# zhan-xu/MoRig

Hardware: AMD Instinct MI355X
Metric: meshes/sec jointnet_motion forward, 4 k-vert synthetic (higher is better)
Workload: dtype f32 (split-fp16: 3x f16 MFMA, f32 accumulate); 1 GPU; jointnet_motion(num_keyframes=5, attn) eval forward, B=64 x 4096-vertex synthetic meshes/GPU, BASELINE.json configs[1]; step=COO->CSR prep + forward, meshes_per_gpu=64, global_batch=64, vertices_per_mesh=4096, parallelism=mesh-sharded dp1, guard_read=deferred, geo_graph=device

## Files before the change

morig_amd/csrc/dma_ring.h:

```cpp
#pragma once
#include "mfma_types.h"

namespace morig {

template <int MT, int NT> struct SplitFrag { f16x8 ah[MT], al[MT], bh[NT], bl[NT]; };

template <int MT, int NT>
__device__ __forceinline__ void load_split_frag(SplitFrag<MT, NT>& f, const char* st, int aoff, int boff, int s2, int hi, int x7) {
    const int sh = ((2 * s2 + hi) ^ x7) * 16, sl = ((4 + 2 * s2 + hi) ^ x7) * 16;
#pragma unroll
    for (int mt = 0; mt < MT; ++mt) {
        f.ah[mt] = *reinterpret_cast<const f16x8*>(st + aoff + mt * 32 * 128 + sh);
        f.al[mt] = *reinterpret_cast<const f16x8*>(st + aoff + mt * 32 * 128 + sl);
    }
#pragma unroll
    for (int nt = 0; nt < NT; ++nt) {
        f.bh[nt] = *reinterpret_cast<const f16x8*>(st + boff + nt * 32 * 128 + sh);
        f.bl[nt] = *reinterpret_cast<const f16x8*>(st + boff + nt * 32 * 128 + sl);
    }
}

template <bool SWAP>
__device__ __forceinline__ void split_mm(const f16x8& x, const f16x8& w, f32x16& c) {
    if constexpr (SWAP) c = __builtin_amdgcn_mfma_f32_32x32x16_f16(w, x, c, 0, 0, 0);
// ... 32 lines not shown
}
__device__ __forceinline__ void dma_piece(const char* base, int c, unsigned o, char* st, int piece) {
    asm volatile("" : "+v"(o));
    __builtin_amdgcn_global_load_lds((glb_void_t*)(base + c * 128 + o), (lds_void_t*)(st + piece * 1024), 16, 0, 0);
}

__device__ __forceinline__ f32x16 acc_zero() {
    f32x16 v;
#pragma unroll
    for (int r = 0; r < 16; ++r) v[r] = 0.f;
    return v;
}
__device__ __forceinline__ f32x16 acc_from_panel(const float* pn, int nt) {
    f32x16 v;
#pragma unroll
    for (int g4 = 0; g4 < 4; ++g4) {
        const f32x4 b4 = *reinterpret_cast<const f32x4*>(pn + nt * 32 + 8 * g4);
#pragma unroll
        for (int q = 0; q < 4; ++q) v[4 * g4 + q] = b4[q];
    }
    return v;
}

}
```

morig_amd/csrc/epilogue_store.h:

```cpp
#pragma once
#include <hip/hip_runtime.h>
#include <type_traits>

namespace morig {

template <int NT, int SLAB = 32, int PAD = 4> struct EpilogueTile {
    static constexpr int CW = NT * 32, LDT = CW + PAD, FLOATS = SLAB * LDT;
};

template <int MT, int NT, bool ALLOW16, class P, int SLAB = 32, int PAD = 4>
__device__ __forceinline__ void store_tile_transposed(const P& p, f32x16 (&acc)[MT][NT], float* T, const int* sseg,
                                                      int rl_base, int row0, int Mlim, int colw0, int lane) {
    static_assert(SLAB == 32 || SLAB == 16, "slab = whole or half MFMA row tile");
    constexpr int CW = EpilogueTile<NT, SLAB, PAD>::CW, LDT = EpilogueTile<NT, SLAB, PAD>::LDT;
    constexpr int VW = 4, LPR = CW / VW, RPI = 64 / LPR;
    constexpr int VW16 = 8, LPR16 = CW / VW16, RPI16 = 64 / LPR16;
    constexpr int NV = ALLOW16 ? 8 : 4;
    const int l31 = lane & 31, hi = lane >> 5;
    const bool y16 = ALLOW16 && p.y16 != 0;
    const bool vec_ok = (reinterpret_cast<size_t>(p.Y) & 15) == 0 && (p.ldy & 3) == 0;
    const int cg = y16 ? (lane % LPR16) * VW16 : (lane % LPR) * VW;
    const int rsel = y16 ? lane / LPR16 : lane / LPR;
    const int col0 = colw0 + cg;
    const int nv = y16 ? VW16 : VW;
// ... 195 lines not shown
        }
    }
    if (ovf) *p.ovf = 1;
}

template <int MT, int NT, class P>
__device__ __forceinline__ void store_tile_regs(const P& p, f32x16 (&acc)[MT][NT], const float* ps, const float* pt,
                                                int rl_base, int row0, int Mlim, int colw0, int cl0, int lane, bool rb_slow) {
#ifdef MORIG_EPI_GENERIC
    store_tile_regs_t<MT, NT, P, false, false, false, false>(p, acc, ps, pt, rl_base, row0, Mlim, colw0, cl0, lane, rb_slow);
#else
    if (rb_slow) { store_tile_regs_t<MT, NT, P, false, false, false, false>(p, acc, ps, pt, rl_base, row0, Mlim, colw0, cl0, lane, rb_slow); return; }
    const int key = (p.y16 != 0 ? 1 : 0) | (p.relu != 0 ? 2 : 0) | (ps != nullptr ? 4 : 0);
#define MORIG_EPI_CASE(K, Y, R, A) case K: store_tile_regs_t<MT, NT, P, true, Y, R, A>(p, acc, ps, pt, rl_base, row0, Mlim, colw0, cl0, lane, false); break;
    switch (key) {
        MORIG_EPI_CASE(0, false, false, false) MORIG_EPI_CASE(1, true, false, false) MORIG_EPI_CASE(2, false, true, false)
        MORIG_EPI_CASE(3, true, true, false) MORIG_EPI_CASE(4, false, false, true) MORIG_EPI_CASE(5, true, false, true)
        MORIG_EPI_CASE(6, false, true, true) MORIG_EPI_CASE(7, true, true, true)
    }
#undef MORIG_EPI_CASE
#endif
}

}
```

morig_amd/csrc/gemm_dma.hip:

```cpp
#include "common.h"
#include "dma_ring.h"
#include "epilogue_store.h"
#include "pool_epilogue.h"
#include <stdlib.h>

namespace morig {

template <int BM, int BN, int NT, int DMA_NS, bool TR = false, bool TAIL = false>
__global__ __launch_bounds__((BM / 64) * (BN / (32 * NT)) * 64) void gemm16_dma_kernel(const GemmDmaParams p) {
    constexpr int MT = 2;
    constexpr int WNW = BN / (32 * NT);
    constexpr int NW = (BM / 64) * WNW;
    constexpr int DMA_STAGE = (BM + BN) * 128;
    constexpr int XJ = BM / 8 / NW, WJ = BN / 8 / NW;
    constexpr int PER_CHUNK = XJ + WJ;
    constexpr int TBYTES = NW * EpilogueTile<NT>::FLOATS * 4;
    constexpr int RING = DMA_NS * DMA_STAGE;
    constexpr int SM0 = (TR || RING > TBYTES) ? RING : TBYTES;
    constexpr int PANEL = TR ? 3 * BN * 4 : 0;
    __shared__ __attribute__((aligned(128))) char smem[SM0 + BM * 4 + PANEL];
    int* sseg = reinterpret_cast<int*>(smem + SM0);
    float* pan = reinterpret_cast<float*>(smem + SM0 + BM * 4);

    const int tid = threadIdx.x, lane = tid & 63, wave = tid >> 6;
    const int l31 = lane & 31, hi = lane >> 5;
    const int wm = wave / WNW, wn = wave % WNW;
    const int lin = xcd_remap(blockIdx.x, gridDim.x);
    const int tn = lin % p.tiles_n, tm = lin / p.tiles_n;
    const int row0 = tm * BM;

#ifdef MORIG_DMA_TRACE
#define DMA_TS(k) do { if ((int)blockIdx.x == (int)(gridDim.x / 2 + 8) && lane == 0) p.trace[(k) * 8 + wave] = __builtin_readcyclecounter(); } while (0)
// ... 79 lines not shown
    const int aoff = (wm * 64 + l31) * 128, boff = BM * 128 + (wn * NT * 32 + l31) * 128;
#ifndef MORIG_2MFMA
    constexpr bool LOHI = true;
#else
    constexpr bool LOHI = false;
#endif
    typedef SplitFrag<MT, NT> Frag;
    auto load_frag = [&](Frag& f, int c, int s2) { load_split_frag(f, smem + (c % DMA_NS) * DMA_STAGE, aoff, boff, s2, hi, x7); };
    auto mma = [&](const Frag& f) { split_mma<TR, LOHI>(f, acc); };
    auto wait_chunk = [&](int c) {
        int younger = nchunk - 1 - c;
        if (younger > DMA_NS - 2) younger = DMA_NS - 2;
        static_assert(DMA_NS >= 2 && DMA_NS <= 4, "ring depth");
        if (younger == 2) asm volatile("s_waitcnt vmcnt(%0)" ::"n"(2 * PER_CHUNK) : "memory");
        else if (younger == 1) asm volatile("s_waitcnt vmcnt(%0)" ::"n"(PER_CHUNK) : "memory");
        else asm volatile("s_waitcnt vmcnt(0)" ::: "memory");
    };
    auto mma_pair = [&](const Frag& f, int mt, int nt0) __attribute__((always_inline)) { split_mma_pair<TR, LOHI>(f, acc, mt, nt0); };
    auto issue_one = [&](int c, int j) __attribute__((always_inline)) {
        char* st = smem + (c % DMA_NS) * DMA_STAGE;
        if (j < XJ) dma_x(st, c, j);
        else dma_w(st, c, j - XJ);
    };
    Frag f0, f1;
    wait_chunk(0);
    if constexpr (TR) asm volatile("s_waitcnt lgkmcnt(0)" ::: "memory");
    __builtin_amdgcn_s_barrier();
    if (DMA_NS - 1 < nchunk) issue(DMA_NS - 1);
    if constexpr (TR) {
#pragma unroll
        for (int nt = 0; nt < NT; ++nt) {
            const f32x16 v = acc_from_panel(pan + wn * NT * 32 + 4 * hi, nt);
#pragma unroll
            for (int mt = 0; mt < MT; ++mt) acc[mt][nt] = v;
        }
    }
    load_frag(f0, 0, 0);
#ifdef MORIG_DMA_BURST
    constexpr bool SPREAD = false;
#else
    constexpr bool SPREAD = (NT == 4 && MT == 2 && PER_CHUNK == 8);
#endif
    for (int c = 0; c < nchunk; ++c) {
        load_frag(f1, c, 1);
        mma(f0);
        const bool more = c + 1 < nchunk;
// ... 31 lines not shown
        if (rfirst >= p.M) return;
        pool_tile<MT, NT>(p, acc, rfirst, colw0, lane);
        return;
    }
    if constexpr (TR) {
        if (p.dbg & 1) { if (acc[0][0][0] == 12345.678f) p.Y[0] = 1.f; return; }
        DMA_TS(2);
        store_tile_regs<MT, NT>(p, acc, p.scale ? pan + BN : nullptr, pan + 2 * BN, wm * 64, row0, p.M, colw0, wn * NT * 32, lane, rb_slow);
        DMA_TS(3);
        return;
    }
    __syncthreads();
    if (p.dbg & 1) { if (acc[0][0][0] == 12345.678f) p.Y[0] = 1.f; return; }
    DMA_TS(2);
    store_tile_transposed<MT, NT, true>(p, acc, reinterpret_cast<float*>(smem) + wave * EpilogueTile<NT>::FLOATS, sseg,
                                        wm * 64, row0, p.M, colw0, lane);
    DMA_TS(3);
#ifdef MORIG_DMA_TRACE
    asm volatile("s_waitcnt vmcnt(0)" ::: "memory");
    DMA_TS(4);
#endif
}

int launch_gemm16_dma(const GemmDmaParams& p0, int tiles_m128, hipStream_t s) {
    GemmDmaParams p = p0;
    p.dbg = debug_flags();
    static const int mode = [] { const char* e = getenv("MORIG_DMA_TILE"); return e ? atoi(e) : 256; }();
    static const int persist = [] { const char* e = getenv("MORIG_DMA_PERSIST"); return e ? (e[0] == '0' ? 0 : 2) : 1; }();
    const bool deep_wide = p.pool != nullptr || (p.K >= 768 && p.N >= 1024);
    const bool vec_ok = p.pool != nullptr ||
                        ((reinterpret_cast<uintptr_t>(p.Y) & 15) == 0 && (p.ldy & 3) == 0 &&
                         (!p.rowbias || ((reinterpret_cast<uintptr_t>(p.rowbias) & 15) == 0 && (p.ld_rowbias & 3) == 0)));
    if (p.Xt && !(mode == 256 && p.N % 256 == 0 && !p.pool)) return MORIG_E_UNSUPPORTED;
    static const int small_tiles = [] { const char* e = getenv("MORIG_DMA_SMALL_TILES"); return e ? atoi(e) : 256; }();
    const bool few_tiles = !p.Xt && p.N % 256 == 0 && (long)cdiv(p.M, 256) * (p.N / 256) <= small_tiles;
    if (!few_tiles && !p.Xt && mode == 256 && p.N % 256 == 0 && p.K > 32 && vec_ok && (persist == 2 || (persist == 1 && deep_wide))) {
        if (!p.pool) prof_retag(K_GEMM16_DMAP);
        return launch_gemm16_dmap(p0, s);
    }
    if (mode == 256 && p.N % 256 == 0 && !few_tiles) {
        p.tiles_n = p.N / 256;
        const int nb = cdiv(p.M, 256) * p.tiles_n;
#ifdef MORIG_DMA_TRACE
        static unsigned long long* trace_buf = [] { void* b = nullptr; return hipMalloc(&b, 64 * 8) == hipSuccess ? (unsigned long long*)b : nullptr; }();
        p.trace = trace_buf;
#endif
        static const bool want_tr = [] { const char* e = getenv("MORIG_GEMM_TR"); return !(e && e[0] == '0'); }();
        const bool tr = want_tr && !p.pool && (reinterpret_cast<uintptr_t>(p.Y) & 15) == 0 && (p.ldy & 3) == 0 &&
                        (!p.rowbias || ((reinterpret_cast<uintptr_t>(p.rowbias) & 15) == 0 && (p.ld_rowbias & 3) == 0));
        static const int shortk = [] { const char* e = getenv("MORIG_DMA_SHORTK"); return e ? atoi(e) : 0; }();
        if (tr && !p.Xt && shortk > 0 && p.K <= shortk && p.N % 128 == 0) {
            p.tiles_n = p.N / 128;
            const int nb128 = cdiv(p.M, 128) * p.tiles_n;
            prof_retag(K_GEMM16_DMA128);
            hipLaunchKernelGGL((gemm16_dma_kernel<128, 128, 2, 2, true>), dim3(nb128), dim3(256), 0, s, p);
            MORIG_LAUNCH_CHECK();
            return MORIG_OK;
        }
        if (p.Xt && !tr) return MORIG_E_UNSUPPORTED;
        if (p.Xt)    hipLaunchKernelGGL((gemm16_dma_kernel<256, 256, 4, 2, true, true>), dim3(nb), dim3(512), 0, s, p);
        else if (tr) hipLaunchKernelGGL((gemm16_dma_kernel<256, 256, 4, 2, true>), dim3(nb), dim3(512), 0, s, p);
        else         hipLaunchKernelGGL((gemm16_dma_kernel<256, 256, 4, 2, false>), dim3(nb), dim3(512), 0, s, p);
#ifdef MORIG_DMA_TRACE
        {
            unsigned long long h[64];
            if (hipStreamSynchronize(s) == hipSuccess && hipMemcpy(h, p.trace, sizeof(h), hipMemcpyDeviceToHost) == hipSuccess) {
                fprintf(stderr, "DMA_TRACE K=%d N=%d:", p.K, p.N);
                for (int w = 0; w < 8; w += 3) { fprintf(stderr, " w%d", w); for (int q = 1; q < 5; ++q) fprintf(stderr, " %lld", (long long)(h[q * 8 + w] - h[(q - 1) * 8 + w])); }
                fprintf(stderr, "\n");
            }
        }
#endif
    } else {
        p.tiles_n = cdiv(p.N, 128);
        prof_retag(K_GEMM16_DMA128);
        hipLaunchKernelGGL((gemm16_dma_kernel<128, 128, 2, 2, false>), dim3(tiles_m128 * p.tiles_n), dim3(256), 0, s, p);
    }
    MORIG_LAUNCH_CHECK();
    return MORIG_OK;
}

}
```

morig_amd/csrc/gemm_dmap.hip:

```cpp
#include "common.h"
#include "dma_ring.h"
#include "epilogue_store.h"
#include "pool_epilogue.h"
#include "pool_runs.h"
#include <stdlib.h>
#include <type_traits>

namespace morig {

struct GemmDmaHot { int M, K, ldx, ldw, tiles_n; const float* X; const float* W; const int* seg; };
typedef __attribute__((address_space(4))) const GemmDmaParams* kernarg_params_t;
template <bool POOL>
__global__ __launch_bounds__(512) void gemm16_dmap_kernel(const GemmDmaParams) {
#if defined(__HIP_DEVICE_COMPILE__)
    kernarg_params_t q = (kernarg_params_t)__builtin_amdgcn_kernarg_segment_ptr();
    asm volatile("" : "+s"(q));
    const GemmDmaHot p = {q->M, q->K, q->ldx, q->ldw, q->tiles_n, q->X, q->W, q->seg};
    constexpr int BM = 256, BN = 256, NT = 4, MT = 2;
    constexpr int WNW = BN / (32 * NT);
    constexpr int NW = (BM / 64) * WNW;
    constexpr int STAGE = (BM + BN) * 128;
    constexpr int XJ = BM / 8 / NW, WJ = BN / 8 / NW;
    constexpr int PANEL = 3 * BN;
    constexpr int PAIR = 2 * NT * 64;
    __shared__ __attribute__((aligned(128))) char smem[2 * STAGE + (POOL ? NW * PAIR * 4 : 2 * PANEL * 4)];
    float* pan = reinterpret_cast<float*>(smem + 2 * STAGE);

    const int tid = threadIdx.x, lane = tid & 63, wave = tid >> 6;
    const int l31 = lane & 31, hi = lane >> 5;
    const int wm = wave / WNW, wn = wave % WNW;

    const int tiles_m = (p.M + BM - 1) / BM;
    const int T = tiles_m * p.tiles_n;
    const int xcd = blockIdx.x & 7, bi = blockIdx.x >> 3, nbx = gridDim.x >> 3;
    TileList tl = {};
    int run_u = 0, run_left = 0;
// ... 91 lines not shown
            asm volatile("" : "+v"(f0.ah[0]), "+v"(f0.al[0]), "+v"(f0.ah[1]), "+v"(f0.al[1]));
            asm volatile("" : "+v"(f0.bh[0]), "+v"(f0.bl[0]), "+v"(f0.bh[1]), "+v"(f0.bl[1]), "+v"(f0.bh[2]), "+v"(f0.bl[2]), "+v"(f0.bh[3]), "+v"(f0.bl[3]));
#else
            load_frag(f0, st ^ 1, 0);
#endif
        }
        unsigned o0 = ox[0], o1 = ox[1], o2 = ox[2], o3 = ox[3];
        if (go && reclamp) { o0 = x_offset(0, nrow0); o1 = x_offset(1, nrow0); o2 = x_offset(2, nrow0); o3 = x_offset(3, nrow0); }
        mma_pair(f1, 0, 0); __builtin_amdgcn_sched_barrier(0);
        if constexpr (go) { dma_x(xb, o0, cc, st, 0); dma_x(xb, o1, cc, st, 1); }
        __builtin_amdgcn_sched_barrier(0);
        mma_pair(f1, 0, 2); __builtin_amdgcn_sched_barrier(0);
        if constexpr (go) { dma_x(xb, o2, cc, st, 2); dma_x(xb, o3, cc, st, 3); }
        __builtin_amdgcn_sched_barrier(0);
        mma_pair(f1, 1, 0); __builtin_amdgcn_sched_barrier(0);
        if constexpr (go) { dma_w(wb, cc, st, 0); dma_w(wb, cc, st, 1); }
        __builtin_amdgcn_sched_barrier(0);
        mma_pair(f1, 1, 2); __builtin_amdgcn_sched_barrier(0);
        if constexpr (go) { dma_w(wb, cc, st, 2); dma_w(wb, cc, st, 3); }
        __builtin_amdgcn_sched_barrier(0);
    };
    typedef std::integral_constant<int, 1> Yes;
    typedef std::integral_constant<int, 0> No;

    int lin = tl.first;
    if constexpr (POOL) {
        lin = pool_run_first_tile(run_u, p.tiles_n, q->run);
        run_left = pool_run_count(run_u, tiles_m, p.tiles_n, q->run) - 1;
    }
    static_assert(NT == 4 && PAIR == 2 * 4 * 64, "the pair is kept as two 16-byte vectors per thread");
    auto pair_ptr = [&](int t) __attribute__((always_inline)) { return reinterpret_cast<f32x4*>(smem + 2 * STAGE) + t; };
    int rseg = -1;
    bool drained = true;
    const int wave_s = __builtin_amdgcn_readfirstlane(wave);
    if constexpr (POOL) {
        pair_ptr(tid)[0] = f32x4{-INFINITY, -INFINITY, -INFINITY, -INFINITY};
        pair_ptr(tid)[512] = f32x4{INFINITY, INFINITY, INFINITY, INFINITY};
    }
    int g = 0;
    {
        const int row0 = (lin / p.tiles_n) * BM;
        const char* xbase = reinterpret_cast<const char*>(p.X + (size_t)row0 * p.ldx);
        const char* wbase = reinterpret_cast<const char*>(p.W + (size_t)((lin % p.tiles_n) * BN) * p.ldw);
#pragma unroll
        for (int j = 0; j < XJ; ++j) dma_x(xbase, x_offset(j, row0), 0, 0, j);
#pragma unroll
// ... 8 lines not shown
    for (int jt = 0; jt < n_my; ++jt) {
        const int tn = lin % p.tiles_n, row0 = (lin / p.tiles_n) * BM;
        const char* xbase = reinterpret_cast<const char*>(p.X + (size_t)row0 * p.ldx);
        const char* wbase = reinterpret_cast<const char*>(p.W + (size_t)(tn * BN) * p.ldw);
#pragma unroll
        for (int j = 0; j < XJ; ++j) ox[j] = x_offset(j, row0);
        bool run_end = true;

        if constexpr (POOL) {
            if (!drained) asm volatile("s_waitcnt vmcnt(0)" ::: "memory");
            asm volatile("s_waitcnt lgkmcnt(0)" ::: "memory");
            drained = false;
        }
        __builtin_amdgcn_s_barrier();
#pragma unroll
        for (int j = 0; j < XJ; ++j) dma_x(xbase, ox[j], 1, (g + 1) & 1, j);
#pragma unroll
        for (int j = 0; j < WJ; ++j) dma_w(wbase, 1, (g + 1) & 1, j);
        if constexpr (POOL) {
#pragma unroll
            for (int mt = 0; mt < MT; ++mt)
#pragma unroll
                for (int nt = 0; nt < NT; ++nt) acc[mt][nt] = acc_zero();
        } else {
            const float* pn = pan + (jt & 1) * PANEL + wn * NT * 32 + 4 * hi;
#pragma unroll
            for (int nt = 0; nt < NT; ++nt) {
                const f32x16 v = acc_from_panel(pn, nt);
#pragma unroll
                for (int mt = 0; mt < MT; ++mt) acc[mt][nt] = v;
            }
        }
        load_frag(f0, g & 1, 0);

#pragma unroll 1
        for (int c = 0; c + 2 < nchunk; ++c) chunk_iter((g + c) & 1, Yes{}, Yes{}, xbase, wbase, c + 2, false, 0);
        {
            int nlin = jt + 1 < n_my ? lin + nbx : lin;
            if constexpr (POOL) {
                run_end = run_left == 0;
                if (!run_end) { nlin = lin + p.tiles_n; --run_left; }
                else if (jt + 1 < n_my) {
                    asm volatile("" : "+s"(q));
                    const int R = q->run;
                    run_u += nbx;
                    nlin = pool_run_first_tile(run_u, p.tiles_n, R);
                    run_left = pool_run_count(run_u, tiles_m, p.tiles_n, R) - 1;
                }
            }
            const int nrow0 = (nlin / p.tiles_n) * BM;
            const char* nxbase = reinterpret_cast<const char*>(p.X + (size_t)nrow0 * p.ldx);
            const char* nwbase = reinterpret_cast<const char*>(p.W + (size_t)((nlin % p.tiles_n) * BN) * p.ldw);
            if constexpr (!POOL) panel_fetch(nlin, slow_next);
            chunk_iter((g + nchunk - 2) & 1, Yes{}, Yes{}, nxbase, nwbase, 0, true, nrow0);
            chunk_iter((g + nchunk - 1) & 1, No{}, No{}, nxbase, nwbase, 0, false, 0);
            lin = nlin;
        }

        if constexpr (!POOL) asm volatile("s_waitcnt vmcnt(0) lgkmcnt(0)" ::: "memory");
        const int colw0 = tn * BN + wn * NT * 32;
        if constexpr (POOL) {
            const int elane = __builtin_amdgcn_mbcnt_hi(~0u, __builtin_amdgcn_mbcnt_lo(~0u, 0u)), ewave = wave_s;
            const int te = ewave * 64 + elane;
            const int ecolw0 = tn * BN + (ewave % WNW) * NT * 32;
            const int rfirst = row0 + (ewave / WNW) * 64;
            f32x4* const pair_mx = pair_ptr(te);
            f32x4* const pair_mn = pair_mx + 512;
            auto drain = [&]() __attribute__((always_inline)) {
                if (!drained) { asm volatile("s_waitcnt vmcnt(0)" ::: "memory"); drained = true; }
            };
            auto load_pe = [&](GemmDmaParams& pe) __attribute__((always_inline)) {
                asm volatile("" : "+s"(q));
                pe.M = q->M; pe.N = q->N; pe.bias = q->bias; pe.scale = q->scale; pe.shift = q->shift; pe.relu = q->relu; pe.seg = q->seg;
                pe.pool = q->pool; pe.ld_pool = q->ld_pool;
            };
            auto flush = [&]() __attribute__((always_inline)) {
                drain();
                GemmDmaParams pe;
// ... 10 lines not shown
            if (rseg >= 0 && !(whole && s0 == rseg)) flush();
            if (whole) {
                const f32x4 vx = *pair_mx, vn = *pair_mn;
                float mx[NT] = {vx[0], vx[1], vx[2], vx[3]}, mn[NT] = {vn[0], vn[1], vn[2], vn[3]};
                pool_reduce_rows<MT, NT>(acc, mx, mn);
                *pair_mx = f32x4{mx[0], mx[1], mx[2], mx[3]};
                *pair_mn = f32x4{mn[0], mn[1], mn[2], mn[3]};
                rseg = s0;
            } else if (rfirst < p.M) {
                drain();
                GemmDmaParams pe;
                load_pe(pe);
                pool_tile_per_element<MT, NT>(pe, acc, rfirst, ecolw0, elane);
            }
            if (run_end && rseg >= 0) flush();
        } else {
            panel_write((jt + 1) & 1);
            asm volatile("" : "+s"(q));
            GemmDmaParams pe;
            pe.M = q->M; pe.N = q->N; pe.scale = q->scale; pe.relu = q->relu;
            pe.rowbias = q->rowbias; pe.ld_rowbias = q->ld_rowbias; pe.seg = q->seg;
            pe.Y = q->Y; pe.ldy = q->ldy; pe.y16 = q->y16; pe.ovf = q->ovf; pe.dbg = q->dbg;
            const float* pn = pan + (jt & 1) * PANEL;
            if (!(pe.dbg & 1))
                store_tile_regs<MT, NT>(pe, acc, pe.scale ? pn + BN : nullptr, pn + 2 * BN, wm * 64, row0, pe.M, colw0, wn * NT * 32, lane,
                                        slow_cur);
            slow_cur = slow_next;
        }
        g += nchunk;
    }
    asm volatile("s_waitcnt vmcnt(0)" ::: "memory");
#endif
}

int launch_gemm16_dmap(const GemmDmaParams& p0, hipStream_t s) {
    GemmDmaParams p = p0;
    p.dbg = debug_flags();
    p.tiles_n = p.N / 256;
    const int T = cdiv(p.M, 256) * p.tiles_n;
    const int grid = persistent_grid(T);
    static const int run_env = [] { const char* e = getenv("MORIG_POOL_RUN"); const int v = e ? atoi(e) : 0; return v < 0 ? 0 : (v > 256 ? 256 : v); }();
    if (!p.pool) p.run = 1;
    else if (run_env > 0) p.run = pool_run_length(cdiv(p.M, 256), p.tiles_n, 0, run_env);
    else p.run = pool_run_length(cdiv(p.M, 256), p.tiles_n, grid, 16);
    if (p.pool) hipLaunchKernelGGL(gemm16_dmap_kernel<true>, dim3(grid), dim3(512), 0, s, p);
    else        hipLaunchKernelGGL(gemm16_dmap_kernel<false>, dim3(grid), dim3(512), 0, s, p);
    MORIG_LAUNCH_CHECK();
    return MORIG_OK;
}

}
```

morig_amd/csrc/launch_core.h:

```cpp
#pragma once

namespace morig {

int cu_count();
void set_reserved_cus(int n);
int reserved_cus();
int persistent_grid(int units);
int debug_flags();

}
```

morig_amd/csrc/prof.hip:

```cpp
#include "common.h"
#include <atomic>
#include <mutex>
#include <stdlib.h>
#include <vector>
#include <string.h>

namespace morig {

static int g_last_hip = 0;
void set_hip_error(hipError_t e) { g_last_hip = (int)e; }

int cu_count() {
    static std::atomic<int> cache[64];
    int dev = 0;
    if (hipGetDevice(&dev) != hipSuccess || dev < 0 || dev >= 64) return 256;
    int n = cache[dev].load();
    if (n == 0) {
        if (hipDeviceGetAttribute(&n, hipDeviceAttributeMultiprocessorCount, dev) != hipSuccess || n <= 0) n = 256;
        cache[dev].store(n);
    }
    return n;
}

static std::atomic<int> g_reserved_cus{0};
// ... 136 lines not shown
    MORIG_HIP_TRY(hipGetDeviceProperties(&p, dev));
    if (cu_count) *cu_count = p.multiProcessorCount;
    if (lds_bytes_per_cu) *lds_bytes_per_cu = (int)p.maxSharedMemoryPerMultiProcessor;
    if (clock_khz) *clock_khz = p.clockRate;
    if (arch && arch_len > 0) { strncpy(arch, p.gcnArchName, arch_len - 1); arch[arch_len - 1] = 0; }
    return strncmp(p.gcnArchName, "gfx950", 6) == 0 ? MORIG_OK : MORIG_E_NODEVICE;
}

int morig_prof_enable(int on) {
    std::lock_guard<std::mutex> lk(g_mu);
    int prev = g_on ? 1 : 0;
    g_on = on != 0;
    return prev;
}

int morig_prof_reset(void) {
    std::lock_guard<std::mutex> lk(g_mu);
    drain_locked();
    for (int k = 0; k < K_COUNT; ++k) { g_ms[k] = g_fl[k] = g_by[k] = 0.0; g_n[k] = 0; }
    return MORIG_OK;
}

const char* morig_prof_name(int kind) { return (kind >= 0 && kind < K_COUNT) ? kNames[kind] : nullptr; }
const char* morig_prof_symbol(int kind) { return (kind >= 0 && kind < K_COUNT) ? kSymbols[kind] : nullptr; }

int morig_prof_collect(int kind, int64_t* launches, double* total_ms, double* flops, double* bytes) {
    if (kind < 0 || kind >= K_COUNT) return MORIG_E_INVALID;
    std::lock_guard<std::mutex> lk(g_mu);
    drain_locked();
    if (launches) *launches = g_n[kind];
    if (total_ms) *total_ms = g_ms[kind];
    if (flops) *flops = g_fl[kind];
    if (bytes) *bytes = g_by[kind];
    return MORIG_OK;
}

}
```

morig_amd/csrc/ubench.hip:

```cpp
#include "common.h"

namespace morig {

template <int MODE>
__global__ __launch_bounds__(512, 2) void ubench_mfma_kernel(int iters, float* out, unsigned seed) {
    unsigned s = seed ^ (blockIdx.x * 9781u + threadIdx.x * 6271u + 1u);
    auto rnd = [&]() { s = s * 1664525u + 1013904223u; return s; };
    f16x8 a[4], b[4];
    for (int i = 0; i < 4; ++i) {
        union { unsigned u[4]; f16x8 v; } ua, ub;
        for (int j = 0; j < 4; ++j) {
            const unsigned r = rnd(), q = rnd();
            ua.u[j] = MODE == 1 ? 0u : ((r & 0x83ff83ffu) | 0x34003400u | ((r >> 3) & 0x0c000c00u));
            ub.u[j] = MODE == 1 ? 0u : ((q & 0x83ff83ffu) | 0x34003400u | ((q >> 3) & 0x0c000c00u));
        }
        a[i] = ua.v; b[i] = ub.v;
    }
    f32x16 c[8];
    for (int i = 0; i < 8; ++i) for (int r = 0; r < 16; ++r) c[i][r] = 0.f;
#pragma unroll 1
    for (int it = 0; it < iters; ++it) {
#pragma unroll
        for (int g = 0; g < 3; ++g)
#pragma unroll
            for (int i = 0; i < 8; ++i) c[i] = __builtin_amdgcn_mfma_f32_32x32x16_f16(a[(i + g) & 3], b[i & 3], c[i], 0, 0, 0);
        if ((it & 63) == 63) for (int i = 0; i < 8; ++i) for (int r = 0; r < 16; ++r) c[i][r] *= 1e-3f;
    }
    float acc = 0.f;
    for (int i = 0; i < 8; ++i) for (int r = 0; r < 16; ++r) acc += c[i][r];
    if (acc == 12345.678f) out[0] = acc;
}

}

using namespace morig;

extern "C" int morig_ubench_mfma(int mode, int iters, int launches, float* scratch, double* flops, void* stream) {
    if (iters <= 0 || launches <= 0 || !scratch) return MORIG_E_INVALID;
    const int ncu = cu_count();
    hipStream_t s = reinterpret_cast<hipStream_t>(stream);
    for (int l = 0; l < launches; ++l) {
        if (mode == 1) hipLaunchKernelGGL(ubench_mfma_kernel<1>, dim3(ncu), dim3(512), 0, s, iters, scratch, 17u + l);
        else           hipLaunchKernelGGL(ubench_mfma_kernel<0>, dim3(ncu), dim3(512), 0, s, iters, scratch, 17u + l);
    }
    MORIG_LAUNCH_CHECK();
    if (flops) *flops = 2.0 * 32 * 32 * 16 * 24.0 * iters * 8.0 * ncu * launches;
    return MORIG_OK;
}
```

Measured before the change: 1475 meshes/s.

## Switch DMA split-fp16 GEMM store paths to 16x16x32 MFMA with register epilogue

```diff
diff --git a/morig_amd/csrc/dma_ring.h b/morig_amd/csrc/dma_ring.h
--- a/morig_amd/csrc/dma_ring.h
+++ b/morig_amd/csrc/dma_ring.h
@@ -78,4 +78,40 @@
     return v;
 }
 
+struct SplitFrag16 { f16x8 xh[2][2], xl[2][2], wh[8], wl[8]; };
+constexpr int SPLIT16_MB = 4, SPLIT16_NB = 8;
+
+__device__ __forceinline__ int split16_slot_hi(int q4, int x7) { return (q4 ^ x7) * 16; }
+__device__ __forceinline__ int split16_slot_lo(int q4, int x7) { return ((4 + q4) ^ x7) * 16; }
+__device__ __forceinline__ void load_split_x16(SplitFrag16& f, const char* st, int aoff, int h, int sh, int sl) {
+#pragma unroll
+    for (int m = 0; m < 2; ++m) {
+        f.xh[h][m] = *reinterpret_cast<const f16x8*>(st + aoff + (2 * h + m) * 16 * 128 + sh);
+        f.xl[h][m] = *reinterpret_cast<const f16x8*>(st + aoff + (2 * h + m) * 16 * 128 + sl);
+    }
 }
+__device__ __forceinline__ void load_split_w16(SplitFrag16& f, const char* st, int boff, int nb, int sh, int sl) {
+    f.wh[nb] = *reinterpret_cast<const f16x8*>(st + boff + nb * 16 * 128 + sh);
+    f.wl[nb] = *reinterpret_cast<const f16x8*>(st + boff + nb * 16 * 128 + sl);
+}
+template <bool SWAP>
+__device__ __forceinline__ void split_mm16(const f16x8& x, const f16x8& w, f32x4& c) {
+    if constexpr (SWAP) c = __builtin_amdgcn_mfma_f32_16x16x32_f16(w, x, c, 0, 0, 0);
+    else                c = __builtin_amdgcn_mfma_f32_16x16x32_f16(x, w, c, 0, 0, 0);
+}
+template <bool SWAP, bool LOHI = true>
+__device__ __forceinline__ void split_mma16_group(const SplitFrag16& f, f32x4 (&acc)[SPLIT16_MB][SPLIT16_NB], int h, int nb0) {
+#pragma unroll
+    for (int t = 0; t < 3; ++t) {
+        if (t == 1 && !LOHI) continue;
+#pragma unroll
+        for (int n = 0; n < 2; ++n)
+#pragma unroll
+            for (int m = 0; m < 2; ++m)
+                split_mm16<SWAP>(t == 0 ? f.xl[h][m] : f.xh[h][m], t == 1 ? f.wl[nb0 + n] : f.wh[nb0 + n], acc[2 * h + m][nb0 + n]);
+    }
+}
+__device__ __forceinline__ f32x4 acc_zero16() { return f32x4{0.f, 0.f, 0.f, 0.f}; }
+__device__ __forceinline__ f32x4 acc_from_panel16(const float* pn, int nb) { return *reinterpret_cast<const f32x4*>(pn + nb * 16); }
+
+}
diff --git a/morig_amd/csrc/epilogue_store.h b/morig_amd/csrc/epilogue_store.h
--- a/morig_amd/csrc/epilogue_store.h
+++ b/morig_amd/csrc/epilogue_store.h
@@ -241,4 +241,106 @@
 #endif
 }
 
-}
+template <class P, bool CT, bool Y16, bool RELU, bool AFF>
+__device__ __forceinline__ void store_tile_regs16_t(const P& p, f32x4 (&acc)[4][8], const float* ps, const float* pt,
+                                                    int rl_base, int row0, int Mlim, int colw0, int cl0, int lane, bool rb_slow) {
+    const int l15 = lane & 15, g = lane >> 4;
+    const bool y16 = CT ? Y16 : (p.y16 != 0);
+    const bool relu = CT ? RELU : (p.relu != 0), aff = CT ? AFF : (ps != nullptr);
+    if (CT) rb_slow = false;
+    bool ovf = false;
+#pragma unroll
+    for (int mb = 0; mb < 4; ++mb) {
+        const int row = row0 + rl_base + mb * 16 + l15;
+        const bool ok = row < Mlim;
+        float* yrow = p.Y + (size_t)(ok ? row : 0) * p.ldy;
+        const float* rbrow = nullptr;
+        if (rb_slow && ok) rbrow = p.rowbias + (size_t)p.seg[row] * p.ld_rowbias;
+        if (!y16) {
+#pragma unroll
+            for (int nb = 0; nb < 8; ++nb) {
+                const int c4 = nb * 16 + 4 * g;
+                f32x4 v = acc[mb][nb];
+                if (rbrow) v += *reinterpret_cast<const f32x4*>(rbrow + colw0 + c4);
+                if (relu) {
+#pragma unroll
+                    for (int q = 0; q < 4; ++q) v[q] = fmaxf(v[q], 0.f);
+                }
+                if (aff) {
+                    const f32x4 s0 = *reinterpret_cast<const f32x4*>(ps + cl0 + c4), t0 = *reinterpret_cast<const f32x4*>(pt + cl0 + c4);
+#pragma unroll
+                    for (int q = 0; q < 4; ++q) v[q] = v[q] * s0[q] + t0[q];
+                }
+                if (!ok) continue;
+                *reinterpret_cast<f32x4*>(yrow + colw0 + c4) = v;
+            }
+        } else {
+#pragma unroll
+            for (int P2 = 0; P2 < 4; ++P2) {
+                float v[8];
+#pragma unroll
+                for (int q = 0; q < 4; ++q) {
+                    const float fa = acc[mb][2 * P2][q], fb = acc[mb][2 * P2 + 1][q];
+                    const auto sw = __builtin_amdgcn_permlane16_swap(__float_as_uint(fa), __float_as_uint(fb), false, false);
+                    const unsigned ua = sw[0], ub = sw[1];
+                    v[q] = __uint_as_float(ua);
+                    v[4 + q] = __uint_as_float(ub);
+                }
+                const int c8 = P2 * 32 + 16 * (g & 1) + 8 * (g >> 1);
+                if (rbrow) {
+                    const f32x4 r0 = *reinterpret_cast<const f32x4*>(rbrow + colw0 + c8);
+                    const f32x4 r1 = *reinterpret_cast<const f32x4*>(rbrow + colw0 + c8 + 4);
+#pragma unroll
+                    for (int q = 0; q < 4; ++q) { v[q] += r0[q]; v[4 + q] += r1[q]; }
+                }
+                if (relu) {
+#pragma unroll
+                    for (int q = 0; q < 8; ++q) v[q] = fmaxf(v[q], 0.f);
+                }
+                if (aff) {
+                    const f32x4 s0 = *reinterpret_cast<const f32x4*>(ps + cl0 + c8), s1 = *reinterpret_cast<const f32x4*>(ps + cl0 + c8 + 4);
+                    const f32x4 t0 = *reinterpret_cast<const f32x4*>(pt + cl0 + c8), t1 = *reinterpret_cast<const f32x4*>(pt + cl0 + c8 + 4);
+#pragma unroll
+                    for (int q = 0; q < 4; ++q) { v[q] = v[q] * s0[q] + t0[q]; v[4 + q] = v[4 + q] * s1[q] + t1[q]; }
+                }
+                if (!ok) continue;
+                const int col = colw0 + c8;
+                typedef __fp16 ep_h2 __attribute__((ext_vector_type(2)));
+                typedef float ep_b32x4 __attribute__((ext_vector_type(4)));
+                ep_b32x4 hw, lw;
+                float am = 0.f;
+#pragma unroll
+                for (int q = 0; q < 8; q += 2) {
+                    const ep_h2 h = __builtin_amdgcn_cvt_pkrtz(v[q], v[q + 1]);
+                    const float hb = __builtin_bit_cast(float, h);
+                    float lb;
+                    asm("v_fma_mixlo_f16 %0, %1, 1.0, -%2 op_sel_hi:[0,0,1]" : "=v"(lb) : "v"(v[q]), "v"(hb));
+                    asm("v_fma_mixhi_f16 %0, %1, 1.0, -%2 op_sel:[0,0,1] op_sel_hi:[0,0,1]" : "+v"(lb) : "v"(v[q + 1]), "v"(hb));
+                    hw[q >> 1] = hb; lw[q >> 1] = lb;
+                    am = fmaxf(am, fmaxf(fabsf(v[q]), fabsf(v[q + 1])));
+                }
+                if (!(am < FP16_RANGE_GUARD)) ovf = true;
+                char* o = reinterpret_cast<char*>(yrow) + (col >> 5) * 128 + (col & 31) * 2;
+                *reinterpret_cast<f16x8*>(o) = __builtin_bit_cast(f16x8, hw);
+                *reinterpret_cast<f16x8*>(o + 64) = __builtin_bit_cast(f16x8, lw);
+            }
+        }
+    }
+    if (ovf) *p.ovf = 1;
+}
+
+template <class P>
+__device__ __forceinline__ void store_tile_regs16(const P& p, f32x4 (&acc)[4][8], const float* ps, const float* pt,
+                                                  int rl_base, int row0, int Mlim, int colw0, int cl0, int lane, bool rb_slow) {
+    if (rb_slow) { store_tile_regs16_t<P, false, false, false, false>(p, acc, ps, pt, rl_base, row0, Mlim, colw0, cl0, lane, rb_slow); return; }
+    const int key = (p.y16 != 0 ? 1 : 0) | (p.relu != 0 ? 2 : 0) | (ps != nullptr ? 4 : 0);
+#define MORIG_EPI_CASE(K, Y, R, A) case K: store_tile_regs16_t<P, true, Y, R, A>(p, acc, ps, pt, rl_base, row0, Mlim, colw0, cl0, lane, false); break;
+    switch (key) {
+        MORIG_EPI_CASE(0, false, false, false) MORIG_EPI_CASE(1, true, false, false) MORIG_EPI_CASE(2, false, true, false)
+        MORIG_EPI_CASE(3, true, true, false) MORIG_EPI_CASE(4, false, false, true) MORIG_EPI_CASE(5, true, false, true)
+        MORIG_EPI_CASE(6, false, true, true) MORIG_EPI_CASE(7, true, true, true)
+    }
+#undef MORIG_EPI_CASE
+}
+
+}
diff --git a/morig_amd/csrc/gemm_dma.hip b/morig_amd/csrc/gemm_dma.hip
--- a/morig_amd/csrc/gemm_dma.hip
+++ b/morig_amd/csrc/gemm_dma.hip
@@ -6,8 +6,9 @@
 
 namespace morig {
 
-template <int BM, int BN, int NT, int DMA_NS, bool TR = false, bool TAIL = false>
+template <int BM, int BN, int NT, int DMA_NS, bool TR = false, bool TAIL = false, int SH = 32>
 __global__ __launch_bounds__((BM / 64) * (BN / (32 * NT)) * 64) void gemm16_dma_kernel(const GemmDmaParams p) {
+    static_assert(SH == 32 || (SH == 16 && TR && NT == 4), "16x16x32: the 64 x 128 wave tile with the register epilogue; every other form is 32x32x16");
     constexpr int MT = 2;
     constexpr int WNW = BN / (32 * NT);
     constexpr int NW = (BM / 64) * WNW;
@@ -133,6 +134,54 @@
         if (j < XJ) dma_x(st, c, j);
         else dma_w(st, c, j - XJ);
     };
+    if constexpr (SH == 16) {
+        static_assert(PER_CHUNK == 8, "the DMA pieces are spread in four pairs");
+        const int q4 = lane >> 4;
+        const int sh16 = split16_slot_hi(q4, (lane >> 1) & 7), sl16 = split16_slot_lo(q4, (lane >> 1) & 7);
+        const int aoff16 = (wm * 64 + (lane & 15)) * 128, boff16 = BM * 128 + (wn * 128 + (lane & 15)) * 128;
+        auto stage = [&](int c) __attribute__((always_inline)) { return smem + (c % DMA_NS) * DMA_STAGE; };
+        f32x4 acc16[SPLIT16_MB][SPLIT16_NB];
+        SplitFrag16 f;
+        wait_chunk(0);
+        asm volatile("s_waitcnt lgkmcnt(0)" ::: "memory");
+        __builtin_amdgcn_s_barrier();
+        if (DMA_NS - 1 < nchunk) issue(DMA_NS - 1);
+#pragma unroll
+        for (int nb = 0; nb < SPLIT16_NB; ++nb) {
+            const f32x4 v = acc_from_panel16(pan + wn * 128 + 4 * q4, nb);
+#pragma unroll
+            for (int mb = 0; mb < SPLIT16_MB; ++mb) acc16[mb][nb] = v;
+        }
+        load_split_x16(f, stage(0), aoff16, 0, sh16, sl16);
+#pragma unroll
+        for (int nb = 0; nb < SPLIT16_NB; ++nb) load_split_w16(f, stage(0), boff16, nb, sh16, sl16);
+        for (int c = 0; c < nchunk; ++c) {
+            load_split_x16(f, stage(c), aoff16, 1, sh16, sl16);
+#pragma unroll
+            for (int nb0 = 0; nb0 < SPLIT16_NB; nb0 += 2) split_mma16_group<true, LOHI>(f, acc16, 0, nb0);
+            const bool more = c + 1 < nchunk;
+            const bool go = more && c + DMA_NS < nchunk;
+            if (more) {
+                wait_chunk(c + 1);
+                asm volatile("s_waitcnt lgkmcnt(0)" ::: "memory");
+                __builtin_amdgcn_s_barrier();
+                load_split_x16(f, stage(c + 1), aoff16, 0, sh16, sl16);
+            }
+#pragma unroll
+            for (int g = 0; g < 4; ++g) {
+                split_mma16_group<true, LOHI>(f, acc16, 1, 2 * g); __builtin_amdgcn_sched_barrier(0);
+                if (more) { load_split_w16(f, stage(c + 1), boff16, 2 * g, sh16, sl16); load_split_w16(f, stage(c + 1), boff16, 2 * g + 1, sh16, sl16); }
+                if (go) { issue_one(c + DMA_NS, 2 * g); issue_one(c + DMA_NS, 2 * g + 1); }
+                __builtin_amdgcn_sched_barrier(0);
+            }
+        }
+        DMA_TS(1);
+        if (p.dbg & 1) { if (acc16[0][0][0] == 12345.678f) p.Y[0] = 1.f; return; }
+        DMA_TS(2);
+        store_tile_regs16(p, acc16, p.scale ? pan + BN : nullptr, pan + 2 * BN, wm * 64, row0, p.M, tn * BN + wn * 128, wn * 128, lane, rb_slow);
+        DMA_TS(3);
+        return;
+    }
     Frag f0, f1;
     wait_chunk(0);
     if constexpr (TR) asm volatile("s_waitcnt lgkmcnt(0)" ::: "memory");
@@ -210,6 +259,20 @@
 #endif
 }
 
+int dma_mfma_shape(int kind) {
+    static const int forced = [] { const char* e = getenv("MORIG_MFMA_SHAPE"); const int v = e ? atoi(e) : 0; return (v == 16 || v == 32) ? v : 0; }();
+    if (forced) return forced;
+    static const int mask = [] { const char* e = getenv("MORIG_MFMA_SHAPE_KINDS"); return e ? atoi(e) : -1; }();
+    if (mask >= 0) return ((mask >> kind) & 1) ? 16 : 32;
+    switch (kind) {
+        case DMA_KIND_F32_OUT:   return 16;
+        case DMA_KIND_TAIL:      return 16;
+        case DMA_KIND_SPLIT_OUT: return 16;
+        case DMA_KIND_PERSIST:   return 16;
+        default:                 return 32;
+    }
+}
+
 int launch_gemm16_dma(const GemmDmaParams& p0, int tiles_m128, hipStream_t s) {
     GemmDmaParams p = p0;
     p.dbg = debug_flags();
@@ -246,7 +309,10 @@
             return MORIG_OK;
         }
         if (p.Xt && !tr) return MORIG_E_UNSUPPORTED;
-        if (p.Xt)    hipLaunchKernelGGL((gemm16_dma_kernel<256, 256, 4, 2, true, true>), dim3(nb), dim3(512), 0, s, p);
+        const int sh = !tr ? 32 : dma_mfma_shape(p.Xt ? DMA_KIND_TAIL : p.y16 ? DMA_KIND_SPLIT_OUT : DMA_KIND_F32_OUT);
+        if (sh == 16 && p.Xt) hipLaunchKernelGGL((gemm16_dma_kernel<256, 256, 4, 2, true, true, 16>), dim3(nb), dim3(512), 0, s, p);
+        else if (sh == 16)    hipLaunchKernelGGL((gemm16_dma_kernel<256, 256, 4, 2, true, false, 16>), dim3(nb), dim3(512), 0, s, p);
+        else if (p.Xt) hipLaunchKernelGGL((gemm16_dma_kernel<256, 256, 4, 2, true, true>), dim3(nb), dim3(512), 0, s, p);
         else if (tr) hipLaunchKernelGGL((gemm16_dma_kernel<256, 256, 4, 2, true>), dim3(nb), dim3(512), 0, s, p);
         else         hipLaunchKernelGGL((gemm16_dma_kernel<256, 256, 4, 2, false>), dim3(nb), dim3(512), 0, s, p);
 #ifdef MORIG_DMA_TRACE
diff --git a/morig_amd/csrc/gemm_dmap.hip b/morig_amd/csrc/gemm_dmap.hip
--- a/morig_amd/csrc/gemm_dmap.hip
+++ b/morig_amd/csrc/gemm_dmap.hip
@@ -10,8 +10,9 @@
 
 struct GemmDmaHot { int M, K, ldx, ldw, tiles_n; const float* X; const float* W; const int* seg; };
 typedef __attribute__((address_space(4))) const GemmDmaParams* kernarg_params_t;
-template <bool POOL>
-__global__ __launch_bounds__(512) void gemm16_dmap_kernel(const GemmDmaParams) {
+template <bool POOL, int SH>
+__device__ __forceinline__ void gemm16_dmap_body() {
+    static_assert(SH == 32 || (SH == 16 && !POOL), "16x16x32: the store launches (register epilogue); pooled launches are 32x32x16");
 #if defined(__HIP_DEVICE_COMPILE__)
     kernarg_params_t q = (kernarg_params_t)__builtin_amdgcn_kernarg_segment_ptr();
     asm volatile("" : "+s"(q));
@@ -149,6 +150,48 @@
     };
     typedef std::integral_constant<int, 1> Yes;
     typedef std::integral_constant<int, 0> No;
+    const int q4 = lane >> 4;
+    const int sh16 = split16_slot_hi(q4, (lane >> 1) & 7), sl16 = split16_slot_lo(q4, (lane >> 1) & 7);
+    const int aoff16 = (wm * 64 + (lane & 15)) * 128, boff16 = BM * 128 + (wn * 128 + (lane & 15)) * 128;
+    f32x4 acc16[SPLIT16_MB][SPLIT16_NB];
+    SplitFrag16 fs;
+    auto load_first16 = [&](int stage) __attribute__((always_inline)) {
+        load_split_x16(fs, smem + stage * STAGE, aoff16, 0, sh16, sl16);
+#pragma unroll
+        for (int nb = 0; nb < SPLIT16_NB; ++nb) load_split_w16(fs, smem + stage * STAGE, boff16, nb, sh16, sl16);
+    };
+    auto chunk_iter16 = [&](int st, auto morec, auto goc, const char* xb, const char* wb, int cc, bool reclamp, int nrow0)
+                            __attribute__((always_inline)) {
+        constexpr bool more = decltype(morec)::value != 0, go = decltype(goc)::value != 0;
+        load_split_x16(fs, smem + st * STAGE, aoff16, 1, sh16, sl16);
+#pragma unroll
+        for (int nb0 = 0; nb0 < SPLIT16_NB; nb0 += 2) split_mma16_group<true>(fs, acc16, 0, nb0);
+        if constexpr (more) {
+            asm volatile("s_waitcnt vmcnt(0)" ::: "memory");
+            asm volatile("s_waitcnt lgkmcnt(0)" ::: "memory");
+            __builtin_amdgcn_s_barrier();
+            load_split_x16(fs, smem + (st ^ 1) * STAGE, aoff16, 0, sh16, sl16);
+        }
+        unsigned o[XJ] = {ox[0], ox[1], ox[2], ox[3]};
+        if (go && reclamp) { o[0] = x_offset(0, nrow0); o[1] = x_offset(1, nrow0); o[2] = x_offset(2, nrow0); o[3] = x_offset(3, nrow0); }
+#pragma unroll
+        for (int g4 = 0; g4 < 4; ++g4) {
+            split_mma16_group<true>(fs, acc16, 1, 2 * g4); __builtin_amdgcn_sched_barrier(0);
+            if constexpr (more) {
+                load_split_w16(fs, smem + (st ^ 1) * STAGE, boff16, 2 * g4, sh16, sl16);
+                load_split_w16(fs, smem + (st ^ 1) * STAGE, boff16, 2 * g4 + 1, sh16, sl16);
+            }
+            if constexpr (go) {
+                if (g4 < 2) { dma_x(xb, o[2 * g4], cc, st, 2 * g4); dma_x(xb, o[2 * g4 + 1], cc, st, 2 * g4 + 1); }
+                else        { dma_w(wb, cc, st, 2 * g4 - 4); dma_w(wb, cc, st, 2 * g4 - 3); }
+            }
+            __builtin_amdgcn_sched_barrier(0);
+        }
+    };
+    auto chunk = [&](int st, auto morec, auto goc, const char* xb, const char* wb, int cc, bool reclamp, int nrow0) __attribute__((always_inline)) {
+        if constexpr (SH == 16) chunk_iter16(st, morec, goc, xb, wb, cc, reclamp, nrow0);
+        else                    chunk_iter(st, morec, goc, xb, wb, cc, reclamp, nrow0);
+    };
 
     int lin = tl.first;
     if constexpr (POOL) {
@@ -203,6 +246,14 @@
             for (int mt = 0; mt < MT; ++mt)
 #pragma unroll
                 for (int nt = 0; nt < NT; ++nt) acc[mt][nt] = acc_zero();
+        } else if constexpr (SH == 16) {
+            const float* pn = pan + (jt & 1) * PANEL + wn * 128 + 4 * q4;
+#pragma unroll
+            for (int nb = 0; nb < SPLIT16_NB; ++nb) {
+                const f32x4 v = acc_from_panel16(pn, nb);
+#pragma unroll
+                for (int mb = 0; mb < SPLIT16_MB; ++mb) acc16[mb][nb] = v;
+            }
         } else {
             const float* pn = pan + (jt & 1) * PANEL + wn * NT * 32 + 4 * hi;
 #pragma unroll
@@ -212,10 +263,11 @@
                 for (int mt = 0; mt < MT; ++mt) acc[mt][nt] = v;
             }
         }
-        load_frag(f0, g & 1, 0);
+        if constexpr (SH == 16) load_first16(g & 1);
+        else                    load_frag(f0, g & 1, 0);
 
 #pragma unroll 1
-        for (int c = 0; c + 2 < nchunk; ++c) chunk_iter((g + c) & 1, Yes{}, Yes{}, xbase, wbase, c + 2, false, 0);
+        for (int c = 0; c + 2 < nchunk; ++c) chunk((g + c) & 1, Yes{}, Yes{}, xbase, wbase, c + 2, false, 0);
         {
             int nlin = jt + 1 < n_my ? lin + nbx : lin;
             if constexpr (POOL) {
@@ -233,8 +285,8 @@
             const char* nxbase = reinterpret_cast<const char*>(p.X + (size_t)nrow0 * p.ldx);
             const char* nwbase = reinterpret_cast<const char*>(p.W + (size_t)((nlin % p.tiles_n) * BN) * p.ldw);
             if constexpr (!POOL) panel_fetch(nlin, slow_next);
-            chunk_iter((g + nchunk - 2) & 1, Yes{}, Yes{}, nxbase, nwbase, 0, true, nrow0);
-            chunk_iter((g + nchunk - 1) & 1, No{}, No{}, nxbase, nwbase, 0, false, 0);
+            chunk((g + nchunk - 2) & 1, Yes{}, Yes{}, nxbase, nwbase, 0, true, nrow0);
+            chunk((g + nchunk - 1) & 1, No{}, No{}, nxbase, nwbase, 0, false, 0);
             lin = nlin;
         }
 
@@ -291,6 +343,10 @@
             pe.rowbias = q->rowbias; pe.ld_rowbias = q->ld_rowbias; pe.seg = q->seg;
             pe.Y = q->Y; pe.ldy = q->ldy; pe.y16 = q->y16; pe.ovf = q->ovf; pe.dbg = q->dbg;
             const float* pn = pan + (jt & 1) * PANEL;
+            if constexpr (SH == 16) {
+                if (!(pe.dbg & 1))
+                    store_tile_regs16(pe, acc16, pe.scale ? pn + BN : nullptr, pn + 2 * BN, wm * 64, row0, pe.M, colw0, wn * NT * 32, lane, slow_cur);
+            } else
             if (!(pe.dbg & 1))
                 store_tile_regs<MT, NT>(pe, acc, pe.scale ? pn + BN : nullptr, pn + 2 * BN, wm * 64, row0, pe.M, colw0, wn * NT * 32, lane,
                                         slow_cur);
@@ -301,6 +357,11 @@
     asm volatile("s_waitcnt vmcnt(0)" ::: "memory");
 #endif
 }
+
+template <bool POOL>
+__global__ __launch_bounds__(512) void gemm16_dmap_kernel(const GemmDmaParams) { gemm16_dmap_body<POOL, 32>(); }
+template <bool POOL, int SH>
+__global__ __launch_bounds__(512) void gemm16_dmap_kernel(const GemmDmaParams) { gemm16_dmap_body<POOL, SH>(); }
 
 int launch_gemm16_dmap(const GemmDmaParams& p0, hipStream_t s) {
     GemmDmaParams p = p0;
@@ -313,6 +374,7 @@
     else if (run_env > 0) p.run = pool_run_length(cdiv(p.M, 256), p.tiles_n, 0, run_env);
     else p.run = pool_run_length(cdiv(p.M, 256), p.tiles_n, grid, 16);
     if (p.pool) hipLaunchKernelGGL(gemm16_dmap_kernel<true>, dim3(grid), dim3(512), 0, s, p);
+    else if (dma_mfma_shape(DMA_KIND_PERSIST) == 16) hipLaunchKernelGGL((gemm16_dmap_kernel<false, 16>), dim3(grid), dim3(512), 0, s, p);
     else        hipLaunchKernelGGL(gemm16_dmap_kernel<false>, dim3(grid), dim3(512), 0, s, p);
     MORIG_LAUNCH_CHECK();
     return MORIG_OK;
diff --git a/morig_amd/csrc/launch_core.h b/morig_amd/csrc/launch_core.h
--- a/morig_amd/csrc/launch_core.h
+++ b/morig_amd/csrc/launch_core.h
@@ -7,5 +7,7 @@
 int reserved_cus();
 int persistent_grid(int units);
 int debug_flags();
+enum { DMA_KIND_F32_OUT, DMA_KIND_TAIL, DMA_KIND_SPLIT_OUT, DMA_KIND_PERSIST };
+int dma_mfma_shape(int kind);
 
 }
diff --git a/morig_amd/csrc/prof.hip b/morig_amd/csrc/prof.hip
--- a/morig_amd/csrc/prof.hip
+++ b/morig_amd/csrc/prof.hip
@@ -182,7 +182,10 @@
 }
 
 const char* morig_prof_name(int kind) { return (kind >= 0 && kind < K_COUNT) ? kNames[kind] : nullptr; }
-const char* morig_prof_symbol(int kind) { return (kind >= 0 && kind < K_COUNT) ? kSymbols[kind] : nullptr; }
+const char* morig_prof_symbol(int kind) {
+    if (kind == K_GEMM16_DMAP && dma_mfma_shape(DMA_KIND_PERSIST) == 16) return "gemm16_dmap_kernel<false, 16>";
+    return (kind >= 0 && kind < K_COUNT) ? kSymbols[kind] : nullptr;
+}
 
 int morig_prof_collect(int kind, int64_t* launches, double* total_ms, double* flops, double* bytes) {
     if (kind < 0 || kind >= K_COUNT) return MORIG_E_INVALID;
diff --git a/morig_amd/csrc/ubench.hip b/morig_amd/csrc/ubench.hip
--- a/morig_amd/csrc/ubench.hip
+++ b/morig_amd/csrc/ubench.hip
@@ -1,6 +1,8 @@
 #include "common.h"
 
 namespace morig {
+
+__device__ __forceinline__ unsigned ubench_h2(unsigned r) { return (r & 0x83ff83ffu) | 0x34003400u | ((r >> 3) & 0x0c000c00u); }
 
 template <int MODE>
 __global__ __launch_bounds__(512, 2) void ubench_mfma_kernel(int iters, float* out, unsigned seed) {
@@ -31,19 +33,148 @@
     if (acc == 12345.678f) out[0] = acc;
 }
 
+template <bool ZERO>
+__global__ __launch_bounds__(512, 2) void ubench_mfma16_kernel(int passes, float* out, unsigned seed) {
+    unsigned s = seed ^ (blockIdx.x * 9781u + threadIdx.x * 6271u + 1u);
+    auto rnd = [&]() { s = s * 1664525u + 1013904223u; return s; };
+    f16x8 a[4], b[4];
+    for (int i = 0; i < 4; ++i) {
+        union { unsigned u[4]; f16x8 v; } ua, ub;
+        for (int j = 0; j < 4; ++j) {
+            const unsigned r = rnd(), q = rnd();
+            ua.u[j] = ZERO ? 0u : ubench_h2(r);
+            ub.u[j] = ZERO ? 0u : ubench_h2(q);
+        }
+        a[i] = ua.v; b[i] = ub.v;
+    }
+    f32x4 c[32];
+    for (int i = 0; i < 32; ++i) for (int r = 0; r < 4; ++r) c[i][r] = 0.f;
+#pragma unroll 1
+    for (int it = 0; it < passes; ++it) {
+#pragma unroll
+        for (int g = 0; g < 3; ++g)
+#pragma unroll
+            for (int i = 0; i < 32; ++i)
+                c[i] = __builtin_amdgcn_mfma_f32_16x16x32_f16(a[(i + g) & 3], b[(i + (i >> 2)) & 3], c[i], 0, 0, 0);
+        if ((it & 31) == 31) for (int i = 0; i < 32; ++i) for (int r = 0; r < 4; ++r) c[i][r] *= 1e-3f;
+    }
+    float acc = 0.f;
+    for (int i = 0; i < 32; ++i) for (int r = 0; r < 4; ++r) acc += c[i][r];
+    if (acc == 12345.678f) out[0] = acc;
+}
+
+constexpr int UBENCH_LDS = 24 * 1024;
+__device__ __forceinline__ void ubench_fill_lds(char* lds, unsigned seed) {
+    unsigned s = seed ^ (blockIdx.x * 9781u + threadIdx.x * 6271u + 1u);
+    for (int i = threadIdx.x; i < UBENCH_LDS / 4; i += 512) {
+        s = s * 1664525u + 1013904223u;
+        reinterpret_cast<unsigned*>(lds)[i] = ubench_h2(s ^ (i * 2654435761u));
+    }
+    __syncthreads();
+}
+__device__ __forceinline__ f16x8 ubench_frag(const char* lp, int i) {
+    asm volatile("" : "+v"(lp));
+    return *reinterpret_cast<const f16x8*>(lp + i * 1024);
+}
+
+__global__ __launch_bounds__(512, 2) void ubench_mfma_lds32_kernel(int iters, float* out, unsigned seed) {
+    __shared__ __attribute__((aligned(128))) char lds[UBENCH_LDS];
+    ubench_fill_lds(lds, seed);
+    const char* lp = lds + (threadIdx.x & 63) * 16;
+    struct Frag { f16x8 ah[2], al[2], bh[4], bl[4]; };
+    auto load = [&](Frag& f, int half) __attribute__((always_inline)) {
+        for (int m = 0; m < 2; ++m) { f.ah[m] = ubench_frag(lp, half * 12 + m); f.al[m] = ubench_frag(lp, half * 12 + 2 + m); }
+        for (int n = 0; n < 4; ++n) { f.bh[n] = ubench_frag(lp, half * 12 + 4 + n); f.bl[n] = ubench_frag(lp, half * 12 + 8 + n); }
+    };
+    f32x16 c[2][4];
+    for (int m = 0; m < 2; ++m) for (int n = 0; n < 4; ++n) for (int r = 0; r < 16; ++r) c[m][n][r] = 0.f;
+    auto mma = [&](const Frag& f) __attribute__((always_inline)) {
+#pragma unroll
+        for (int m = 0; m < 2; ++m)
+#pragma unroll
+            for (int n0 = 0; n0 < 4; n0 += 2) {
+                c[m][n0]     = __builtin_amdgcn_mfma_f32_32x32x16_f16(f.al[m], f.bh[n0],     c[m][n0],     0, 0, 0);
+                c[m][n0 + 1] = __builtin_amdgcn_mfma_f32_32x32x16_f16(f.al[m], f.bh[n0 + 1], c[m][n0 + 1], 0, 0, 0);
+                c[m][n0]     = __builtin_amdgcn_mfma_f32_32x32x16_f16(f.ah[m], f.bl[n0],     c[m][n0],     0, 0, 0);
+                c[m][n0 + 1] = __builtin_amdgcn_mfma_f32_32x32x16_f16(f.ah[m], f.bl[n0 + 1], c[m][n0 + 1], 0, 0, 0);
+                c[m][n0]     = __builtin_amdgcn_mfma_f32_32x32x16_f16(f.ah[m], f.bh[n0],     c[m][n0],     0, 0, 0);
+                c[m][n0 + 1] = __builtin_amdgcn_mfma_f32_32x32x16_f16(f.ah[m], f.bh[n0 + 1], c[m][n0 + 1], 0, 0, 0);
+            }
+    };
+    Frag f0, f1;
+    load(f0, 0);
+#pragma unroll 1
+    for (int it = 0; it < iters; it += 2) {
+        load(f1, 1);
+        mma(f0);
+        load(f0, 0);
+        mma(f1);
+        if ((it & 62) == 62) for (int m = 0; m < 2; ++m) for (int n = 0; n < 4; ++n) for (int r = 0; r < 16; ++r) c[m][n][r] *= 1e-3f;
+    }
+    float acc = (float)f0.ah[0][0];
+    for (int m = 0; m < 2; ++m) for (int n = 0; n < 4; ++n) for (int r = 0; r < 16; ++r) acc += c[m][n][r];
+    if (acc == 12345.678f) out[0] = acc;
+}
+
+__global__ __launch_bounds__(512, 2) void ubench_mfma_lds16_kernel(int passes, float* out, unsigned seed) {
+    __shared__ __attribute__((aligned(128))) char lds[UBENCH_LDS];
+    ubench_fill_lds(lds, seed);
+    const char* lp = lds + (threadIdx.x & 63) * 16;
+    f16x8 xh[2][2], xl[2][2], wh[8], wl[8];
+    auto load_x = [&](int half) __attribute__((always_inline)) {
+        for (int m = 0; m < 2; ++m) { xh[half][m] = ubench_frag(lp, half * 4 + m); xl[half][m] = ubench_frag(lp, half * 4 + 2 + m); }
+    };
+    auto load_w = [&](int n) __attribute__((always_inline)) { wh[n] = ubench_frag(lp, 8 + n); wl[n] = ubench_frag(lp, 16 + n); };
+    f32x4 c[4][8];
+    for (int m = 0; m < 4; ++m) for (int n = 0; n < 8; ++n) for (int r = 0; r < 4; ++r) c[m][n][r] = 0.f;
+    auto mma_half = [&](int half, auto reload) __attribute__((always_inline)) {
+#pragma unroll
+        for (int n = 0; n < 8; ++n) {
+#pragma unroll
+            for (int m = 0; m < 2; ++m) c[2 * half + m][n] = __builtin_amdgcn_mfma_f32_16x16x32_f16(xl[half][m], wh[n], c[2 * half + m][n], 0, 0, 0);
+#pragma unroll
+            for (int m = 0; m < 2; ++m) c[2 * half + m][n] = __builtin_amdgcn_mfma_f32_16x16x32_f16(xh[half][m], wl[n], c[2 * half + m][n], 0, 0, 0);
+#pragma unroll
+            for (int m = 0; m < 2; ++m) c[2 * half + m][n] = __builtin_amdgcn_mfma_f32_16x16x32_f16(xh[half][m], wh[n], c[2 * half + m][n], 0, 0, 0);
+            if constexpr (decltype(reload)::value) load_w(n);
+        }
+    };
+    load_x(0);
+    for (int n = 0; n < 8; ++n) load_w(n);
+#pragma unroll 1
+    for (int it = 0; it < passes; ++it) {
+        load_x(1);
+        mma_half(0, std::false_type{});
+        load_x(0);
+        mma_half(1, std::true_type{});
+        if ((it & 31) == 31) for (int m = 0; m < 4; ++m) for (int n = 0; n < 8; ++n) for (int r = 0; r < 4; ++r) c[m][n][r] *= 1e-3f;
+    }
+    float acc = (float)xh[0][0][0] + (float)wh[0][0];
+    for (int m = 0; m < 4; ++m) for (int n = 0; n < 8; ++n) for (int r = 0; r < 4; ++r) acc += c[m][n][r];
+    if (acc == 12345.678f) out[0] = acc;
+}
+
 }
 
 using namespace morig;
 
 extern "C" int morig_ubench_mfma(int mode, int iters, int launches, float* scratch, double* flops, void* stream) {
     if (iters <= 0 || launches <= 0 || !scratch) return MORIG_E_INVALID;
+    if (mode < 0 || mode > 5) return MORIG_E_INVALID;
     const int ncu = cu_count();
     hipStream_t s = reinterpret_cast<hipStream_t>(stream);
+    const int passes = (iters + 1) / 2;
     for (int l = 0; l < launches; ++l) {
-        if (mode == 1) hipLaunchKernelGGL(ubench_mfma_kernel<1>, dim3(ncu), dim3(512), 0, s, iters, scratch, 17u + l);
-        else           hipLaunchKernelGGL(ubench_mfma_kernel<0>, dim3(ncu), dim3(512), 0, s, iters, scratch, 17u + l);
+        switch (mode) {
+            case 1:  hipLaunchKernelGGL(ubench_mfma_kernel<1>, dim3(ncu), dim3(512), 0, s, iters, scratch, 17u + l); break;
+            case 2:  hipLaunchKernelGGL(ubench_mfma16_kernel<false>, dim3(ncu), dim3(512), 0, s, passes, scratch, 17u + l); break;
+            case 3:  hipLaunchKernelGGL(ubench_mfma16_kernel<true>, dim3(ncu), dim3(512), 0, s, passes, scratch, 17u + l); break;
+            case 4:  hipLaunchKernelGGL(ubench_mfma_lds32_kernel, dim3(ncu), dim3(512), 0, s, 2 * passes, scratch, 17u + l); break;
+            case 5:  hipLaunchKernelGGL(ubench_mfma_lds16_kernel, dim3(ncu), dim3(512), 0, s, passes, scratch, 17u + l); break;
+            default: hipLaunchKernelGGL(ubench_mfma_kernel<0>, dim3(ncu), dim3(512), 0, s, iters, scratch, 17u + l); break;
+        }
     }
     MORIG_LAUNCH_CHECK();
-    if (flops) *flops = 2.0 * 32 * 32 * 16 * 24.0 * iters * 8.0 * ncu * launches;
+    if (flops) *flops = 2.0 * 32 * 32 * 16 * 24.0 * (mode >= 2 ? 2 * passes : iters) * 8.0 * ncu * launches;
     return MORIG_OK;
 }
```

Result: no change. 1488 meshes/s, median of 6 (+0.9%).
